# Diamondfan/CTC_pytorch

Hardware: AMD Instinct MI355X
Metric: acoustic frames/sec/GPU (train) + utterances/sec beam-decode (`decode` object), TIMIT 4x320 BiLSTM (higher is better)
Workload: dtype f32 via bf16x3 split-operand MFMA (f32 accumulate); 1 GPU; cfg2: 4x320 BiLSTM + BN + Linear(62) + CTC, B=32/GPU, T=800, F=40, dropout 0.1, Adam; global_batch=32, seq_len=800, parallelism=dp1, full_length_utterances=True, sync_bn=False

## Files before the change

ctc_pytorch_amd/_lib.py:

```python
import ctypes
import glob
import os
import subprocess

import torch

_HERE = os.path.dirname(os.path.abspath(__file__))
_CSRC = os.path.join(_HERE, "csrc")
SO_PATH = os.environ.get("CTCN_LIBCTCN") or os.path.join(_HERE, "libctcn.so")
_lib = None

c_void_p, c_int, c_float, c_double, c_size_t, c_u64 = (ctypes.c_void_p, ctypes.c_int, ctypes.c_float,
                                                      ctypes.c_double, ctypes.c_size_t, ctypes.c_uint64)

P, I, F, D, Z, U = c_void_p, c_int, c_float, c_double, c_size_t, c_u64
_SIGS = {
    "ctcn_version": (I, []),
    "ctcn_last_error": (ctypes.c_char_p, []),
    "ctcn_device_cus": (I, []),
    "ctcn_device_xcds": (I, []),
    "ctcn_set_option": (I, [ctypes.c_char_p, I]),
    "ctcn_get_option": (I, [ctypes.c_char_p]),
    "ctcn_option_name": (ctypes.c_char_p, [I]),
    "ctcn_set_status_buffer": (I, [P]),
    "ctcn_gemm": (I, [I, I, I, I, I, P, I, P, I, P, I, F, I, P, Z, P]),
    "ctcn_transpose01": (I, [P, P, I, I, I, P]),
    "ctcn_copy_strided4": (I, [P, P, I, I, I, I, Z, Z, Z, Z, P]),
    "ctcn_relu_fwd": (I, [P, P, Z, P]),
    "ctcn_relu_bwd": (I, [P, P, P, Z, P]),
    "ctcn_maxpool2d_fwd": (I, [P, P, P, Z, I, I, I, I, P]),
    "ctcn_maxpool2d_bwd": (I, [P, P, P, Z, I, I, I, I, P]),
    "ctcn_rnn_scratch_bytes": (Z, [I, I, I, I]),
    "ctcn_rnn_fwd": (I, [I, I, I, I, I, I, P, P, P, P, P, P, P, P, I, P, Z, P]),
    "ctcn_rnn_fwd_dropout": (I, [I, I, I, I, I, I, P, P, P, P, P, P, P, P, P, F, U, U, I, P, Z, P]),
    "ctcn_rnn_bwd": (I, [I, I, I, I, I, I, P, P, P, P, P, P, P, P, P, P, P, P, P, P, F, I, P, P, Z, P]),
    "ctcn_rnn_bwd_dropout": (I, [I, I, I, I, I, I, P, P, P, P, P, P, P, P, P, P, P, P, P, P, F, I, P, P, Z, P, F, U, U, P]),
    "ctcn_rnn_bwd_weights": (I, [I, I, I, I, I, I, P, P, P, P, P, P, P, P, F, I, ctypes.c_uint, P, Z, P]),
    "ctcn_bn_ws_bytes": (Z, [I, I, I]),
    "ctcn_bn_fwd_train": (I, [P, P, P, P, P, P, P, P, I, I, I, F, F, I, P, Z, P, P]),
    "ctcn_bn_fwd_eval": (I, [P, P, P, P, P, P, I, I, I, F, I, P]),
    "ctcn_bn_fwd_sums": (I, [P, P, I, I, I, P, Z, P]),
    "ctcn_bn_fwd_finish": (I, [P, P, P, P, P, P, P, P, P, D, I, I, I, F, F, I, P, P]),
    "ctcn_bn_bwd_sums": (I, [P, P, P, P, P, P, I, I, I, I, P, Z, P]),
    "ctcn_bn_bwd_finish": (I, [P, P, P, P, P, P, P, P, P, P, P, D, I, I, I, I, F, P, Z, P]),
    "ctcn_bn_bwd": (I, [P, P, P, P, P, P, P, P, P, I, I, I, I, F, P, Z, P]),
    "ctcn_bn_fwd_train_dropout": (I, [P, P, P, P, P, P, P, P, I, I, I, F, F, I, P, Z, P, P, F, U, U]),
    "ctcn_bn_bwd_dropout": (I, [P, P, P, P, P, P, P, P, P, I, I, I, I, F, P, Z, P, F, U, U]),
    "ctcn_dropout": (I, [P, P, Z, F, U, U, P]),
    "ctcn_conv2d_ws_bytes": (Z, [I] * 11),
    "ctcn_conv2d_fwd": (I, [P, P, P, P] + [I] * 11 + [P]),
    "ctcn_conv2d_bwd": (I, [P, P, P, P, P, P] + [I] * 11 + [F, P, Z, P]),
# ... 31 lines not shown
    "ctcn_diag_squat": (I, [I, I, I, ctypes.c_uint, P]),
    "ctcn_diag_pipeline_chunks": (I, [I, I, I, I, I, I, I, I, ctypes.c_uint]),
    "ctcn_rnn_last_kernel": (ctypes.c_char_p, [I]),
    "ctcn_levenshtein": (ctypes.c_longlong, [P, ctypes.c_longlong, P, ctypes.c_longlong]),
    "ctcn_join_tokens": (ctypes.c_longlong, [P, ctypes.c_longlong, P, I, P, P, P, I, I, P, ctypes.c_longlong, P]),
    "ctcn_beam_ws_bytes": (Z, [I, I, I, I]),
    "ctcn_beam_decode": (I, [P, I, P, P, D, I, I, P, P, P, P, I, I, I, P, Z, P]),
    "ctcn_beam_decode_nbest": (I, [P, I, P, P, D, I, I, I, P, P, P, P, P, I, I, I, P, Z, P]),
}


class RnnCall(ctypes.Structure):
    _fields_ = [("drop_p", ctypes.c_float), ("drop_seed", ctypes.c_uint64), ("drop_offset", ctypes.c_uint64), ("y_drop", ctypes.c_void_p),
                ("dy_tmp", ctypes.c_void_p), ("side_stream", ctypes.c_void_p), ("side_event", ctypes.c_void_p), ("side_ws", ctypes.c_void_p),
                ("side_ws_bytes", ctypes.c_size_t), ("xcd_allow", ctypes.c_uint), ("prelaunch_event", ctypes.c_void_p), ("status", ctypes.c_void_p),
                ("launched", ctypes.POINTER(ctypes.c_char_p))]


def sources():
    return sorted(glob.glob(os.path.join(_CSRC, "*.hip")))


def build(force=False, verbose=False):
    from concurrent.futures import ThreadPoolExecutor
    srcs = sources()
    hdrs = glob.glob(os.path.join(_CSRC, "*.h")) + [os.path.join(os.path.dirname(_HERE), "include", "ctcn.h")]
    hipcc = os.environ.get("HIPCC", "/opt/rocm/bin/hipcc")
    objdir = os.path.join(_CSRC, "_obj")
    os.makedirs(objdir, exist_ok=True)
    hdr_time = max(os.path.getmtime(h) for h in hdrs)
    flags = ["--offload-arch=gfx950", "-O3", "-std=c++17", "-fPIC"]
# ... 96 lines not shown
```

ctc_pytorch_amd/csrc/common.h:

```cpp
#pragma once
#include <hip/hip_runtime.h>
#include <stdarg.h>
#include <stdint.h>
#include <stdio.h>
#include <string.h>

#include "../../include/ctcn.h"

void ctcn_set_error(const char *fmt, ...);
int *ctcn_status_word(void);
int ctcn_opt_rnn_persistent(void);
int ctcn_transpose01_pair(const float *in0, const float *in1, float *out0, float *out1, int A, int B, int C, void *stream);
struct GemmPlanes {
  const float *A = nullptr; int lda = 0, M = 0, Ka = 0, transA = 0; void *ws_a = nullptr, *st_a = nullptr; bool a_valid = false;
  const float *B = nullptr; int ldb = 0, N = 0, Kb = 0, transB = 0, shift = 0; void *ws_b = nullptr, *st_b = nullptr; const void *bh = nullptr; bool b_valid = false;
  bool same_a = false, same_b = false;
};
int ctcn_gemm_on_xcds(int transA, int transB, int M, int N, int K, const float *A, int lda, const float *B, int ldb, float *C,
                      int ldc, float beta, int precision, void *ws, size_t ws_bytes, void *stream, unsigned xcd_allow, GemmPlanes *planes = nullptr);
int ctcn_gemm_shift_b(int M, int N, int K, const float *A, int lda, const float *B, int ldb, float *C, int ldc, float beta, int precision,
                      void *ws, size_t ws_bytes, void *stream, unsigned xcd_allow, int shift, GemmPlanes *planes = nullptr);
int ctcn_opt_handoff(void);
int ctcn_opt_poll_depth(void);
int ctcn_opt_bwd_scatter(void);
int ctcn_opt_handoff_tags(void);
int ctcn_opt_side_split_wgs(void);
int ctcn_opt_gemm_big_tiles(void);
int ctcn_opt_recurrence_only(void);

#define CTCN_REQUIRE(cond, ...)          \
  do {                                   \
    if (!(cond)) {                       \
// ... 65 lines not shown
```

ctc_pytorch_amd/csrc/core.hip:

```cpp
#include "common.h"

static thread_local char g_err[512] = "";

void ctcn_set_error(const char *fmt, ...) {
  va_list ap;
  va_start(ap, fmt);
  vsnprintf(g_err, sizeof(g_err), fmt, ap);
  va_end(ap);
}

extern "C" int ctcn_version(void) { return 100; }
extern "C" const char *ctcn_last_error(void) { return g_err; }
extern "C" int ctcn_device_cus(void) {
  int dev = 0, n = 0;
  if (hipGetDevice(&dev) != hipSuccess) return -1;
  if (hipDeviceGetAttribute(&n, hipDeviceAttributeMultiprocessorCount, dev) != hipSuccess) return -1;
  return n;
}

static int g_opt_rnn_persistent = 1;
static int g_opt_handoff = 1;
static int g_opt_poll_depth = 2;
static int g_opt_recurrence_only = 0;
static int g_opt_bwd_scatter = 1;
// ... 19 lines not shown
static int g_opt_conv_dbg = 0;
static int g_opt_rnn_rsv_nt = 0;
static int g_opt_gemm_bf16_single = 0;
static int g_opt_xcd_interleave = 1;
static int g_opt_bn_rows4 = 1;
static int g_opt_tn_splits_force = 0;
static int g_opt_tn_splits_xcd = 1;
static int g_opt_beam_generic_threads = 0;
static int g_opt_beam_bitonic = 1;
static int g_opt_beam_cand_global = 0;
static int g_opt_beam_occ2 = 0;
static int g_opt_beam_fast = 1;
static int g_opt_rnn_slow_items = 0;
static int g_opt_rnn_slow_exchange = 0;
static int g_opt_xcd_interleave_force = 0;
static int *g_status_dev = nullptr;

struct OptionRow { const char *name; int *var; int (*norm)(int); };
static const OptionRow k_options[] = {
  {"rnn_persistent", &g_opt_rnn_persistent, [](int value) -> int { return value; }},
  {"handoff", &g_opt_handoff, [](int value) -> int { return value; }},
  {"poll_depth", &g_opt_poll_depth, [](int value) -> int { return value; }},
  {"rnn_recurrence_only", &g_opt_recurrence_only, [](int value) -> int { return value ? 1 : 0; }},
  {"bwd_scatter", &g_opt_bwd_scatter, [](int value) -> int { return value ? 1 : 0; }},
  {"handoff_tags", &g_opt_handoff_tags, [](int value) -> int { return value ? 1 : 0; }},
  {"side_split_wgs", &g_opt_side_split_wgs, [](int value) -> int { return value < 1 ? 1 : (value > 16 ? 16 : value); }},
  {"gemm_big_tiles", &g_opt_gemm_big_tiles, [](int value) -> int { return value ? 1 : 0; }},
  {"beam_fast", &g_opt_beam_fast, [](int value) -> int { return value ? 1 : 0; }},
  {"conv_dbg", &g_opt_conv_dbg, [](int value) -> int { return value & 7; }},
  {"rnn_rsv_nt", &g_opt_rnn_rsv_nt, [](int value) -> int { return value ? 1 : 0; }},
// ... 12 lines not shown
  {"bwd_item_gather", &g_opt_bwd_item_gather, [](int value) -> int { return value < 0 ? 0 : (value > 2 ? 2 : value); }},
  {"bwd_poll_delay", &g_opt_bwd_poll_delay, [](int value) -> int { return value < 0 ? -1 : (value > 256 ? 256 : value); }},
  {"conv_mfma", &g_opt_conv_mfma, [](int value) -> int { return value ? 1 : 0; }},
  {"edit_wave", &g_opt_edit_wave, [](int value) -> int { return value ? 1 : 0; }},
  {"gemm_tn", &g_opt_gemm_tn, [](int value) -> int { return value != 0; }},
  {"rnn_fused_dropout", &g_opt_rnn_fused_dropout, [](int value) -> int { return value != 0; }},
  {"tag_poll_delay", &g_opt_tag_poll_delay, [](int value) -> int { return value < 0 ? 0 : (value > 64 ? 64 : value); }},
  {"rnn_fwd_tagged", &g_opt_rnn_fwd_tagged, [](int value) -> int { return value ? 1 : 0; }},
  {"rnn_mixed_slices", &g_opt_rnn_mixed_slices, [](int value) -> int { return value ? 1 : 0; }},
  {"gemm_pingpong", &g_opt_gemm_pingpong, [](int value) -> int { return value ? 1 : 0; }},
  {"gemm_a_inline", &g_opt_gemm_a_inline, [](int value) -> int { return value ? 1 : 0; }},
  {"gemm_dbg", &g_opt_gemm_dbg, [](int value) -> int { return value; }},
  {"gemm_tile256", &g_opt_gemm_tile256, [](int value) -> int { return value ? 1 : 0; }},
  {"xcd_interleave_force", &g_opt_xcd_interleave_force, [](int value) -> int { return value ? 1 : 0; }},
  {"rnn_slow_exchange", &g_opt_rnn_slow_exchange, [](int value) -> int { return value < 0 ? 0 : (value > 4096 ? 4096 : value); }},
  {"rnn_slow_items", &g_opt_rnn_slow_items, [](int value) -> int { return value < 0 ? 0 : (value > 4096 ? 4096 : value); }},
};
static const int k_noptions = (int)(sizeof(k_options) / sizeof(k_options[0]));
static const OptionRow *find_option(const char *name) {
  if (name)
    for (int i = 0; i < k_noptions; ++i)
      if (!strcmp(name, k_options[i].name)) return &k_options[i];
  return nullptr;
}
extern "C" int ctcn_set_option(const char *name, int value) {
  if (const OptionRow *o = find_option(name)) { *o->var = o->norm(value); return CTCN_OK; }
  ctcn_set_error("ctcn_set_option: unknown option %s", name ? name : "(null)");
  return CTCN_EINVAL;
}
extern "C" int ctcn_get_option(const char *name) {
// ... 15 lines not shown
```

ctc_pytorch_amd/csrc/gemm.hip:

```cpp
#include <algorithm>
#include <type_traits>

#include "common.h"

namespace {

constexpr int BM = 128, BN = 128, BK = 16, PAD = 4;

__device__ __forceinline__ void g2r_kc(const float *__restrict__ src, int ld, int r0, int R, int k0, int Kend,
                                       bool vec, int tid, float (&reg)[8]) {
#pragma unroll
  for (int j = 0; j < 2; ++j) {
    const int idx = tid + 256 * j;
    const int r = idx >> 2, kq = (idx & 3) * 4;
    const int gr = r0 + r, gk = k0 + kq;
    const float *p = src + (size_t)gr * ld + gk;
    if (vec && gr < R && gk + 3 < Kend) {
      const float4 v = *reinterpret_cast<const float4 *>(p);
      reg[4 * j + 0] = v.x; reg[4 * j + 1] = v.y; reg[4 * j + 2] = v.z; reg[4 * j + 3] = v.w;
    } else {
#pragma unroll
      for (int c = 0; c < 4; ++c) reg[4 * j + c] = (gr < R && gk + c < Kend) ? p[c] : 0.0f;
    }
  }
// ... 1623 lines not shown

}

static bool tn_eligible(int transA, int transB, int M, int N, int K, const float *A, int lda, const float *B, int ldb, int precision, const void *ws,
                        size_t ws_bytes) {
  return precision == 1 && transA && !transB && ws && ws_bytes >= 1024 && ctcn_get_option("gemm_tn") != 0 && M >= 128 && N >= 32 && K >= 1024 &&
         M % 4 == 0 && N % 4 == 0 && lda % 4 == 0 && ldb % 4 == 0 && ((uintptr_t)A & 15) == 0 && ((uintptr_t)B & 15) == 0 &&
         lda < (1 << 24) && ldb < (1 << 24);
}
static int gemm_core(int transA, int transB, int M, int N, int K, const float *A, int lda, const float *B, int ldb, float *C,
                     int ldc, float beta, int precision, void *ws, size_t ws_bytes, void *stream, unsigned xcd_allow, GemmPlanes *planes, int b_shift) {
  GemmPlanes scratch_planes;
  GemmPlanes &pl = planes ? *planes : scratch_planes;
  const bool want_same_a = pl.same_a, want_same_b = pl.same_b;
  pl.same_a = pl.same_b = false;
  CTCN_REQUIRE(precision == 0 || precision == 1, "ctcn_gemm: precision %d (0 = f32 MFMA, 1 = bf16x3 split MFMA)", precision);
  CTCN_REQUIRE(M > 0 && N > 0 && K >= 0, "ctcn_gemm: bad dims M=%d N=%d K=%d", M, N, K);
  CTCN_REQUIRE(A && B && C, "ctcn_gemm: null pointer");
  CTCN_REQUIRE(lda >= (transA ? M : K) && ldb >= (transB ? K : N) && ldc >= N, "ctcn_gemm: leading dim too small");
  hipStream_t st = (hipStream_t)stream;
  const int tiles_m = ceil_div(M, BM), tiles_n = ceil_div(N, BN);
  const int nt = tiles_m * tiles_n;
  int splits = 1;
  if (nt < 256 && K >= 512 && ws && ws_bytes >= (size_t)2 * M * N * sizeof(float)) {
    splits = ceil_div(512, nt);
    splits = min(splits, K / 256);
    splits = min(splits, (int)(ws_bytes / ((size_t)M * N * sizeof(float))));
    if (splits < 2) splits = 1;
  }
  int kchunk = K;
// ... 27 lines not shown
      int nq = 0;
      auto split = [&](const float *src, int ld, bool contraction_major, int rows, unsigned short *hi, unsigned short *lo, int shift) {
        if (!contraction_major) {
          const size_t total = (size_t)rows * (Kp / 4);
          hipLaunchKernelGGL(split_rows_kernel, dim3((unsigned)std::min((size_t)8192, ceil_div_z(total, 256))), dim3(256), 0, st, src, ld, rows, K, Kp, hi, lo);
        } else {
          if (xcd_allow)
            hipLaunchKernelGGL(split_transpose_queue_kernel, dim3(ctcn_opt_side_split_wgs() * ctcn_device_cus()), dim3(256), 0, st, src, ld, K, rows, Kp, hi, lo, ceil_div(rows, 64),
                               ceil_div(Kp, 64), xcd_allow, queue + (++nq), shift);
          else
            hipLaunchKernelGGL(split_transpose_kernel, dim3(ceil_div(rows, 64), ceil_div(Kp, 64)), dim3(256), 0, st, src, ld, K, rows, Kp, hi, lo, shift);
        }
      };
      const bool same_a = want_same_a && pl.a_valid && pl.A == A && pl.lda == lda && pl.M == M && pl.Ka == K && pl.transA == transA && pl.ws_a == ws &&
                          pl.st_a == (void *)st;
      const bool same_b = want_same_b && pl.b_valid && pl.B == B && pl.ldb == ldb && pl.N == N && pl.Kb == K && pl.transB == transB && pl.shift == b_shift &&
                          pl.ws_b == ws && pl.st_b == (void *)st && pl.bh == (const void *)bh;
      pl.B = B; pl.ldb = ldb; pl.N = N; pl.Kb = K; pl.transB = transB; pl.shift = b_shift; pl.ws_b = ws;
      pl.st_b = (void *)st; pl.bh = (const void *)bh; pl.b_valid = true;
      const int wnt256 = (N % 256 == 0 || (N > 512 && ceil_div(N, 256) * 256 - N <= N / 8)) ? 2 : 1;
      const bool use256 = !xcd_allow && ctcn_get_option("gemm_tile256") != 0 && M >= 1024 && N >= 96 &&
                          (long)ceil_div(M, 256) * ceil_div(N, 128 * wnt256) * 4 >= (long)ctcn_device_cus() * 3;
      const bool a_inline = use256 && !same_a && !transA && ctcn_get_option("gemm_a_inline") != 0 && K >= 32 && K % 4 == 0 && lda % 4 == 0 &&
                            ((uintptr_t)A & 15) == 0 && ceil_div(N, 128 * wnt256) <= 5;
      if (a_inline) {
        pl.a_valid = false;
        if (!same_b) split(B, ldb, transB == 0, N, bh, bl, b_shift);
        CTCN_LAUNCH_CHECK();
        const int lrc = wnt256 == 2 ? launch_planes256_af32<2>(st, M, N, K, Kp, A, lda, bh, bl, C, ldc, beta)
                                    : launch_planes256_af32<1>(st, M, N, K, Kp, A, lda, bh, bl, C, ldc, beta);
        if (lrc) return lrc;
        CTCN_LAUNCH_CHECK();
        return CTCN_OK;
      }
// ... 83 lines not shown
  } else {
    if (transA) { if (transB) LAUNCH(gemm_bf16x3_kernel, true, true); else LAUNCH(gemm_bf16x3_kernel, true, false); }
    else        { if (transB) LAUNCH(gemm_bf16x3_kernel, false, true); else LAUNCH(gemm_bf16x3_kernel, false, false); }
  }
#undef LAUNCH
  CTCN_LAUNCH_CHECK();
  if (splits > 1) {
    const size_t total = (size_t)M * N;
    const int blocks = (int)min((size_t)2048, ceil_div_z(total, 256));
    hipLaunchKernelGGL(splitk_reduce_kernel, dim3(blocks), dim3(256), 0, st, (const float *)ws, C, M, N, ldc, splits, beta);
    CTCN_LAUNCH_CHECK();
  }
  return CTCN_OK;
}

int ctcn_gemm_on_xcds(int transA, int transB, int M, int N, int K, const float *A, int lda, const float *B, int ldb, float *C,
                      int ldc, float beta, int precision, void *ws, size_t ws_bytes, void *stream, unsigned xcd_allow, GemmPlanes *planes) {
  return gemm_core(transA, transB, M, N, K, A, lda, B, ldb, C, ldc, beta, precision, ws, ws_bytes, stream, xcd_allow, planes, 0);
}

int ctcn_gemm_shift_b(int M, int N, int K, const float *A, int lda, const float *B, int ldb, float *C, int ldc, float beta, int precision,
                      void *ws, size_t ws_bytes, void *stream, unsigned xcd_allow, int shift, GemmPlanes *planes) {
  const int as = shift < 0 ? -shift : shift;
  CTCN_REQUIRE(as < K, "ctcn_gemm_shift_b: |shift| %d >= K %d", as, K);
  const int Kp = ceil_div(K, PBK) * PBK;
  const size_t plane_bytes = align_up(2 * ((size_t)M * Kp + (size_t)N * Kp) * sizeof(unsigned short), 256);
  const bool plane = precision == 1 && K >= 64 && ws && ws_bytes >= plane_bytes + 1024 &&
                     !tn_eligible(1, 0, M, N, K - as, A, lda, B, ldb, precision, ws, ws_bytes);
  if (!plane) {
    if (planes) planes->same_a = false;
// ... 67 lines not shown
```

ctc_pytorch_amd/csrc/rnn.hip:

```cpp
#include <algorithm>
#include <stdlib.h>

#include <atomic>

#include "common.h"
#include <type_traits>

namespace {

__device__ __forceinline__ float act_sigmoid(float x) { return __builtin_amdgcn_rcpf(1.0f + __builtin_amdgcn_exp2f(-1.4426950408889634f * x)); }
__device__ __forceinline__ float act_tanh(float x) {
  const float e = __builtin_amdgcn_exp2f(-2.8853900817779268f * fabsf(x));
  return copysignf((1.0f - e) * __builtin_amdgcn_rcpf(1.0f + e), x);
}

typedef __bf16 bf16x8_t __attribute__((ext_vector_type(8)));
union Bf16Pack { u32x4 u; bf16x8_t v; };
__device__ __forceinline__ void split8(const f32x4 &a, const f32x4 &b, bf16x8_t &hi, bf16x8_t &lo) {
  unsigned h[8], l[8];
#pragma unroll
  for (int e = 0; e < 8; ++e) {
    const float x = e < 4 ? a[e] : b[e - 4];
    h[e] = f2bf(x);
    l[e] = f2bf(x - __uint_as_float(h[e] << 16));
// ... 2377 lines not shown
                            float *aux, int precision, void *ws, size_t ws_bytes, void *stream) {
  return ctcn_rnn_fwd_ex(cell, T, B, I, H, dirs, x, w_ih0, w_hh0, w_ih1, w_hh1, y, gates, aux, precision, ws, ws_bytes, stream, nullptr);
}
extern "C" int ctcn_rnn_fwd_dropout(int cell, int T, int B, int I, int H, int dirs, const float *x, const float *w_ih0, const float *w_hh0,
                                    const float *w_ih1, const float *w_hh1, float *y, float *gates, float *aux, float *y_drop, float p, uint64_t seed,
                                    uint64_t offset, int precision, void *ws, size_t ws_bytes, void *stream) {
  CTCN_REQUIRE(y_drop && p >= 0.0f && p < 1.0f, "ctcn_rnn_fwd_dropout: y_drop NULL or p=%f outside [0,1)", (double)p);
  ctcn_rnn_call c = {};
  c.y_drop = y_drop; c.drop_p = p; c.drop_seed = seed; c.drop_offset = offset;
  return ctcn_rnn_fwd_ex(cell, T, B, I, H, dirs, x, w_ih0, w_hh0, w_ih1, w_hh1, y, gates, aux, precision, ws, ws_bytes, stream, &c);
}

static int rnn_bwd_gemms(int cell, int T, int B, int I, int H, int dirs, const float *x, const float *w_ih0, const float *w_ih1,
                         const float *y, const float *gates, const float *aux, float *dx, float *dw_ih0, float *dw_hh0, float *dw_ih1,
                         float *dw_hh1, float beta_w, int precision, bool weights, unsigned xcd_allow, void *ws, size_t ws_bytes,
                         void *stream) {
  const int G = gates_of(cell), GH = G * H, TB = T * B;
  const float *w_ih[2] = {w_ih0, w_ih1};
  float *dw_ih[2] = {dw_ih0, dw_ih1};
  float *dw_hh[2] = {dw_hh0, dw_hh1};
  GemmPlanes pl;
  bool dx_done = false;
  if (dx && dirs == 2) {
    StackedWih s;
    if (int rc = stack_w_ih(w_ih0, w_ih1, GH, I, ws, ws_bytes, (hipStream_t)stream, s)) return rc;
    if (s.w) {
      if (int rc = ctcn_gemm_on_xcds(0, 0, TB, I, 2 * GH, gates, 2 * GH, s.w, I, dx, I, 0.0f, precision, s.ws, s.ws_bytes, stream, xcd_allow)) return rc;
      dx_done = true;
    }
  }
  for (int d = 0; d < dirs; ++d) {
    const float *da = gates + (size_t)d * GH;
    const int ldg = dirs * GH;
    int rc;
    if (dx && !dx_done) {
      rc = ctcn_gemm_on_xcds(0, 0, TB, I, GH, da, ldg, w_ih[d], I, dx, I, d == 0 ? 0.0f : 1.0f, precision, ws, ws_bytes, stream, xcd_allow);
      if (rc) return rc;
    }
    if (!weights || !dw_ih[d]) continue;
    rc = ctcn_gemm_on_xcds(1, 0, GH, I, TB, da, ldg, x, I, dw_ih[d], I, beta_w, precision, ws, ws_bytes, stream, xcd_allow, &pl);
    if (rc) return rc;
    const int Kh = (T - 1) * B;
// ... 105 lines not shown
    if (done) note_kernel(1, "rnn_bwd_scatter", c.call);
  }
  return CTCN_OK;
}

static int bwd_per_timestep(BwdCall &c) {
  if (int rc = materialise_dropped_dy(c)) return rc;
  CTCN_HIP(hipMemsetAsync(c.a.state, 0, (size_t)c.B * c.dirs * c.H * sizeof(float), c.st()));
  const int kq4 = pick_kq4(c.GH, 16, 1, 5);
  note_kernel(1, "rnn_bwd_step", c.call);
  for (int s = 0; s < c.T; ++s) {
    c.a.step = s;
    launch_bwd(kq4, c.grid, c.st(), c.a);
  }
  return CTCN_OK;
}

extern "C" int ctcn_rnn_bwd_ex(int cell, int T, int B, int I, int H, int dirs, const float *x, const float *w_ih0,
                               const float *w_hh0, const float *w_ih1, const float *w_hh1, const float *y,
                               float *gates, float *aux, const float *dy, float *dx, float *dw_ih0, float *dw_hh0,
                               float *dw_ih1, float *dw_hh1, float beta_w, int precision, void *scratch, void *ws,
                               size_t ws_bytes, void *stream, const ctcn_rnn_call *call_p) {
  const ctcn_rnn_call &call = call_p ? *call_p : k_plain_call;
  CTCN_REQUIRE(!call.dy_tmp || (call.drop_p >= 0.0f && call.drop_p < 1.0f), "ctcn_rnn_bwd_ex: dropout p=%f outside [0,1)", (double)call.drop_p);
  CTCN_REQUIRE(cell >= 0 && cell <= 2, "ctcn_rnn_bwd: unknown cell %d", cell);
  CTCN_REQUIRE(T > 0 && B > 0 && I > 0 && H > 0 && (dirs == 1 || dirs == 2), "ctcn_rnn_bwd: bad dims");
  if (H % 4 != 0) { ctcn_set_error("ctcn_rnn_bwd: hidden size %d must be a multiple of 4", H); return CTCN_EUNSUPPORTED; }
  CTCN_REQUIRE(x && w_ih0 && w_hh0 && y && gates && dy && scratch, "ctcn_rnn_bwd: null pointer");
  CTCN_REQUIRE((dw_ih0 != nullptr) == (dw_hh0 != nullptr), "ctcn_rnn_bwd: dw_ih0 / dw_hh0 must both be given or both be NULL (weights deferred to ctcn_rnn_bwd_weights)");
  CTCN_REQUIRE(dirs == 1 || (w_ih1 && w_hh1 && (!dw_ih0 || (dw_ih1 && dw_hh1))), "ctcn_rnn_bwd: null pointer (reverse direction)");
// ... 1 lines not shown
  CTCN_REQUIRE((uintptr_t)gates % 16 == 0 && (uintptr_t)scratch % 16 == 0 && (cell == CTCN_CELL_TANH || (uintptr_t)aux % 16 == 0),
               "ctcn_rnn_bwd: gates / aux / scratch must be 16-byte aligned");
  BwdCall c = {cell, T, B, I, H, dirs, precision, dy, ws, ws_bytes, stream, call};
  c.G = gates_of(cell); c.GH = c.G * H;
  const int GH = c.GH;
  c.grid = dim3(ceil_div(H, 16), dirs, ceil_div(B, 16));
  c.status = call.status ? call.status : ctcn_status_word();
  c.fits32 = (size_t)T * B * dirs * GH * sizeof(float) < ((size_t)1 << 32);
  c.dy_dropped = call.dy_tmp == nullptr;
  c.prelaunch_event = call.prelaunch_event;
  c.nxd = ctcn_opt_handoff() ? ctcn_device_xcds() : 1;
  c.persistent = ctcn_opt_rnn_persistent() != 0; c.bwd_scatter = ctcn_opt_bwd_scatter() != 0; c.fused_dropout = ctcn_get_option("rnn_fused_dropout") != 0;
  c.handoff_tags = ctcn_opt_handoff_tags(); c.item_gather = ctcn_get_option("bwd_item_gather"); c.rsv_nt = ctcn_get_option("rnn_rsv_nt");
  c.poll_delay = ctcn_get_option("bwd_poll_delay"); c.slow_items = ctcn_get_option("rnn_slow_items"); c.slow_exchange = ctcn_get_option("rnn_slow_exchange");

  float *whhT = (float *)scratch;
  if (dirs == 2) {
    if (int rc = ctcn_transpose01_pair(w_hh0, w_hh1, whhT, whhT + (size_t)GH * H, GH, H, 1, stream)) return rc;
  } else if (int rc = ctcn_transpose01(w_hh0, whhT, GH, H, 1, stream)) {
    return rc;
  }
  RnnArgs &a = c.a;
  a.cell = cell; a.T = T; a.B = B; a.H = H; a.D = dirs; a.G = c.G; a.step = 0;
  a.w0 = whhT; a.w1 = whhT + (size_t)GH * H; a.y = const_cast<float *>(y); a.gates = gates; a.aux = aux; a.dy = dy;
  a.state = (float *)((char *)scratch + align_up((size_t)dirs * GH * H * sizeof(float), 256));

  bool done = false;
  if (c.persistent && T > 1) {
    const BwdPlan p = bwd_choose_formulation(c);
    Handoff h;
    if (p.feasible && carve_handoff(ws, ws_bytes, p.hx_bytes, p.fl_bytes, h))
      for (int mode = c.nxd > 1 ? 1 : 0; mode >= 0 && !done; --mode)
        if (int rc = bwd_try_persistent(c, p, h, mode, done)) return rc;
    if (!done)
      log_fallback("ctcn_rnn_bwd", T, B, H, dirs, !c.fits32 ? "a reserve tensor of 4 GB or more"
                                                       : (ceil_div(GH, 256) > 8 ? "gate width G*H above 2048" : "not co-resident / workspace too small"));
  }
  record_prelaunch(c);
  if (!done)
    if (int rc = bwd_per_timestep(c)) return rc;
  CTCN_LAUNCH_CHECK();

  if (ctcn_opt_recurrence_only()) return CTCN_OK;
  return rnn_bwd_gemms(cell, T, B, I, H, dirs, x, w_ih0, w_ih1, y, gates, aux, dx, dw_ih0, dw_hh0, dw_ih1, dw_hh1, beta_w, precision,
                       dw_ih0 != nullptr, 0u, ws, ws_bytes, stream);
}

extern "C" int ctcn_rnn_bwd_weights(int cell, int T, int B, int I, int H, int dirs, const float *x, const float *y, const float *gates,
                                    const float *aux, float *dw_ih0, float *dw_hh0, float *dw_ih1, float *dw_hh1, float beta_w,
                                    int precision, unsigned xcd_allow, void *ws, size_t ws_bytes, void *stream) {
  CTCN_REQUIRE(cell >= 0 && cell <= 2, "ctcn_rnn_bwd_weights: unknown cell %d", cell);
  CTCN_REQUIRE(T > 0 && B > 0 && I > 0 && H > 0 && (dirs == 1 || dirs == 2), "ctcn_rnn_bwd_weights: bad dims");
  CTCN_REQUIRE(x && y && gates && (dw_ih0 != nullptr) == (dw_hh0 != nullptr) && (dirs == 1 || (dw_ih1 != nullptr) == (dw_hh1 != nullptr)) &&
                   (dw_ih0 || (dirs == 2 && dw_ih1)), "ctcn_rnn_bwd_weights: null pointer");
  CTCN_REQUIRE(cell != CTCN_CELL_GRU || aux, "ctcn_rnn_bwd_weights: aux (d of the GRU n-gate) required");
  if (ctcn_opt_recurrence_only()) return CTCN_OK;
  return rnn_bwd_gemms(cell, T, B, I, H, dirs, x, nullptr, nullptr, y, gates, aux, nullptr, dw_ih0, dw_hh0, dw_ih1, dw_hh1, beta_w,
                       precision, true, xcd_allow, ws, ws_bytes, stream);
}

// ... 20 lines not shown
```

ctc_pytorch_amd/ops.py:

```python
import collections
import ctypes
import os
import numpy as np

import torch

from . import _lib

CELL = {"lstm": 0, "gru": 1, "tanh": 2}
GATES = {0: 4, 1: 3, 2: 1}

def _precision_from_env():
    v = os.environ.get("CTCN_PRECISION", "1").strip()
    if v not in ("0", "1"):
        raise ValueError("CTCN_PRECISION must be 0 (exact f32 MFMA) or 1 (bf16x3 split-operand MFMA), got %r" % v)
    return int(v)


DEFAULT_PRECISION = _precision_from_env()
_precision = [DEFAULT_PRECISION]


def set_precision(p):
    if int(p) not in (0, 1):
# ... 359 lines not shown
        piped = _side["enabled"] and _side["fwd_overlap"] and allow != 0 and dirs == 2 and T * B * H >= _side["min_items"]
        call = _lib.RnnCall()
        call.status = _lib.status_word(dev).data_ptr()
        if piped:
            st = _side_stream(dev)
            ev = _prelaunch_event(dev)
            w2, wp2, wn2 = _ws(x, tag="side")
            call.side_stream, call.side_event, call.side_ws, call.side_ws_bytes, call.xcd_allow = st.cuda_stream, ev.cuda_event, w2.data_ptr(), wn2, allow
        ctx.drop = None
        y_drop = None
        if training and drop_p > 0.0:
            y_drop = torch.empty_like(y)
            seed, off = _next_dropout_stream(y.numel())
            ctx.drop = (float(drop_p), seed, off)
            call.y_drop, call.drop_p, call.drop_seed, call.drop_offset = y_drop.data_ptr(), float(drop_p), seed, off
        launched = ctypes.c_char_p(None)
        call.launched = ctypes.pointer(launched)
        _lib.check(L.ctcn_rnn_fwd_ex(cell, T, B, I, H, dirs, _ptr(x), _ptr(ws[0]), _ptr(ws[1]), _ptr(ws[2]), _ptr(ws[3]),
                                     _ptr(y), _ptr(gates), _ptr(aux), get_precision(), wp, wn, _lib.stream_ptr(), ctypes.byref(call)), "rnn_fwd_ex")
        _count_kernel(launched.value)
        if T > 1 and B > 16 and (launched.value or b"") == b"rnn_fwd_step" and get_option("rnn_persistent"):
            _fallback_shapes.add((cell, H, dirs, B))
        if _debug_note[0] is not None:
            _debug_note[0]("rnn_fwd", dict(I=int(I), x=x.data_ptr(), gates=gates.data_ptr(), aux=aux.data_ptr() if aux is not None else 0, y=y.data_ptr(),
                                           y_drop=y_drop.data_ptr() if y_drop is not None else 0, ws=w.data_ptr(), w_ih=ws[0].data_ptr(), w_hh=ws[1].data_ptr()),
                           dict(x=x, y=y, gates=gates, aux=aux, y_drop=y_drop, w_ih=(ws[0], ws[2])))
        if piped:
            torch.cuda.current_stream(dev).wait_stream(st)
            for t in (x, gates, ws[0], ws[2]):
                if t is not None:
                    t.record_stream(st)
        ctx.cell, ctx.dims, ctx.has_aux = cell, (T, B, I, H, dirs), aux is not None
        ctx.early_ok = not _chunking[0]
        ctx.consumed = False
        ctx.counted = any(ctx.needs_input_grad)
        if ctx.counted:
            key = (dev.type, dev.index)
            _side["live"][key] = _side["live"].get(key, 0) + 1
        saved = [x, y, gates] + ([aux] if aux is not None else []) + [t for t in ws if t is not None]
        ctx.save_for_backward(*saved)
        return y if y_drop is None else y_drop

    @staticmethod
# ... 48 lines not shown
        small_split = (not side and not split_dirs and not chunk and into_flat and _side["enabled"] and _side["small_split"] and dirs == 2 and T > 1
                       and key not in _side["deferred"] and T * B * H < SMALL_SPLIT_MAX_ITEMS)
        if small_split:
            split_dirs = True
        above, ev = _side["deferred"].pop(key, None), None
        call = _lib.RnnCall()
        call.status = _lib.status_word(dev).data_ptr()
        if above is not None:
            ev = _prelaunch_event(dev)
            call.prelaunch_event = ev.cuda_event
        gd = None
        if ctx.drop is not None:
            p_, seed_, off_ = ctx.drop
            gd = torch.empty_like(gy)
            call.dy_tmp, call.drop_p, call.drop_seed, call.drop_offset = gd.data_ptr(), p_, seed_, off_
        launched = ctypes.c_char_p(None)
        call.launched = ctypes.pointer(launched)
        try:
            _lib.check(L.ctcn_rnn_bwd_ex(cell, T, B, I, H, dirs, _ptr(x), _ptr(w_ih0), _ptr(w_hh0), _ptr(w_ih1), _ptr(w_hh1),
                                         _ptr(y), _ptr(gates), _ptr(aux), _ptr(gy), _ptr(dx),
                                         null if (side or split_dirs) else _ptr(d_ih0), null if (side or split_dirs) else _ptr(d_hh0),
                                         null if (side or split_dirs) else _ptr(d_ih1), null if (side or split_dirs) else _ptr(d_hh1),
                                         1.0 if into_flat else 0.0, get_precision(), _ptr(scratch), wp, wn, _lib.stream_ptr(), ctypes.byref(call)), "rnn_bwd_ex")
        except Exception:
            if above is not None:
                _side["deferred"][key] = above
            raise
        _count_kernel(launched.value)
        if T > 1 and B > 16 and (launched.value or b"") == b"rnn_bwd_step" and get_option("rnn_persistent"):
            _fallback_shapes.add((cell, H, dirs, B))
# ... 836 lines not shown
```

include/ctcn.h:

```cpp
#ifndef CTCN_H
#define CTCN_H
#include <stddef.h>
#include <stdint.h>
#ifdef __cplusplus
extern "C" {
#endif

#define CTCN_OK 0
#define CTCN_EINVAL (-1)
#define CTCN_EHIP (-2)
#define CTCN_EUNSUPPORTED (-3)
#define CTCN_EWORKSPACE (-4)

#define CTCN_REDUCTION_NONE 0
#define CTCN_REDUCTION_MEAN 1
#define CTCN_REDUCTION_SUM 2

#define CTCN_CELL_LSTM 0
#define CTCN_CELL_GRU 1
#define CTCN_CELL_TANH 2

int ctcn_version(void);
const char *ctcn_last_error(void);
int ctcn_device_cus(void);
// ... 29 lines not shown
int ctcn_rnn_bwd_dropout(int cell, int T, int B, int I, int H, int dirs, const float *x, const float *w_ih0, const float *w_hh0,
                         const float *w_ih1, const float *w_hh1, const float *y, float *gates, float *aux, const float *dy, float *dx,
                         float *dw_ih0, float *dw_hh0, float *dw_ih1, float *dw_hh1, float beta_w, int precision, void *scratch, void *ws,
                         size_t ws_bytes, void *stream, float p, uint64_t seed, uint64_t offset, float *dy_tmp);
typedef struct ctcn_rnn_call {
  float drop_p;
  uint64_t drop_seed, drop_offset;
  float *y_drop;
  float *dy_tmp;
  void *side_stream, *side_event, *side_ws;
  size_t side_ws_bytes;
  unsigned xcd_allow;
  void *prelaunch_event;
  int *status;
  const char **launched;
} ctcn_rnn_call;
int ctcn_rnn_fwd_ex(int cell, int T, int B, int I, int H, int dirs, const float *x, const float *w_ih0, const float *w_hh0,
                    const float *w_ih1, const float *w_hh1, float *y, float *gates, float *aux, int precision, void *ws, size_t ws_bytes,
                    void *stream, const ctcn_rnn_call *call);
int ctcn_rnn_bwd_ex(int cell, int T, int B, int I, int H, int dirs, const float *x, const float *w_ih0, const float *w_hh0,
                    const float *w_ih1, const float *w_hh1, const float *y, float *gates, float *aux, const float *dy, float *dx,
                    float *dw_ih0, float *dw_hh0, float *dw_ih1, float *dw_hh1, float beta_w, int precision, void *scratch, void *ws,
                    size_t ws_bytes, void *stream, const ctcn_rnn_call *call);
int ctcn_rnn_bwd_weights(int cell, int T, int B, int I, int H, int dirs, const float *x, const float *y,
                         const float *gates, const float *aux, float *dw_ih0, float *dw_hh0, float *dw_ih1,
                         float *dw_hh1, float beta_w, int precision, unsigned xcd_allow, void *ws, size_t ws_bytes,
                         void *stream);

size_t ctcn_bn_ws_bytes(int outer, int C, int inner);
int ctcn_bn_fwd_train(const float *x, float *y, const float *gamma, const float *beta, float *running_mean,
                      float *running_var, float *save_mean, float *save_rstd, int outer, int C, int inner,
// ... 119 lines not shown
```

Measured before the change: 1.969 million frames/s.

## Precompute backward RNN weight transforms on side stream during forward

Adds a bwd-prep entry point that runs on a side stream during the forward pass. It transposes W_hh and splits the stacked W_ih into bf16 hi/lo planes. The backward pass then uses these prepared buffers through new ctcn_rnn_call fields, and the dx GEMM takes the external B planes, so the transpose and split work leaves the backward critical path. The prepared buffers are reused only when the weight tensor versions are unchanged. The cost is extra allocations per layer, a side-stream sync after the forward call, and more memory held between forward and backward.

New measurement: 1.969 million frames/s (median of 2 runs). About the same (-0.0%).

```diff
diff --git a/ctc_pytorch_amd/_lib.py b/ctc_pytorch_amd/_lib.py
--- a/ctc_pytorch_amd/_lib.py
+++ b/ctc_pytorch_amd/_lib.py
@@ -35,6 +35,8 @@
     "ctcn_rnn_fwd_dropout": (I, [I, I, I, I, I, I, P, P, P, P, P, P, P, P, P, F, U, U, I, P, Z, P]),
     "ctcn_rnn_bwd": (I, [I, I, I, I, I, I, P, P, P, P, P, P, P, P, P, P, P, P, P, P, F, I, P, P, Z, P]),
     "ctcn_rnn_bwd_dropout": (I, [I, I, I, I, I, I, P, P, P, P, P, P, P, P, P, P, P, P, P, P, F, I, P, P, Z, P, F, U, U, P]),
+    "ctcn_rnn_bwd_prep_bytes": (Z, [I, I, I, I, I]),
+    "ctcn_rnn_bwd_prep": (I, [I, I, I, I, P, P, P, P, P, P, P]),
     "ctcn_rnn_bwd_weights": (I, [I, I, I, I, I, I, P, P, P, P, P, P, P, P, F, I, ctypes.c_uint, P, Z, P]),
     "ctcn_bn_ws_bytes": (Z, [I, I, I]),
     "ctcn_bn_fwd_train": (I, [P, P, P, P, P, P, P, P, I, I, I, F, F, I, P, Z, P, P]),
@@ -96,7 +98,7 @@
     _fields_ = [("drop_p", ctypes.c_float), ("drop_seed", ctypes.c_uint64), ("drop_offset", ctypes.c_uint64), ("y_drop", ctypes.c_void_p),
                 ("dy_tmp", ctypes.c_void_p), ("side_stream", ctypes.c_void_p), ("side_event", ctypes.c_void_p), ("side_ws", ctypes.c_void_p),
                 ("side_ws_bytes", ctypes.c_size_t), ("xcd_allow", ctypes.c_uint), ("prelaunch_event", ctypes.c_void_p), ("status", ctypes.c_void_p),
-                ("launched", ctypes.POINTER(ctypes.c_char_p))]
+                ("launched", ctypes.POINTER(ctypes.c_char_p)), ("whh_t", ctypes.c_void_p), ("wih_planes", ctypes.c_void_p)]
 
 
 def sources():
diff --git a/ctc_pytorch_amd/csrc/common.h b/ctc_pytorch_amd/csrc/common.h
--- a/ctc_pytorch_amd/csrc/common.h
+++ b/ctc_pytorch_amd/csrc/common.h
@@ -15,7 +15,10 @@
   const float *A = nullptr; int lda = 0, M = 0, Ka = 0, transA = 0; void *ws_a = nullptr, *st_a = nullptr; bool a_valid = false;
   const float *B = nullptr; int ldb = 0, N = 0, Kb = 0, transB = 0, shift = 0; void *ws_b = nullptr, *st_b = nullptr; const void *bh = nullptr; bool b_valid = false;
   bool same_a = false, same_b = false;
+  const unsigned short *ext_bh = nullptr, *ext_bl = nullptr;
 };
+size_t ctcn_gemm_b_plane_elems(int N, int K);
+int ctcn_gemm_split_b(const float *B, int ldb, int N, int K, unsigned short *hi, unsigned short *lo, void *stream);
 int ctcn_gemm_on_xcds(int transA, int transB, int M, int N, int K, const float *A, int lda, const float *B, int ldb, float *C,
                       int ldc, float beta, int precision, void *ws, size_t ws_bytes, void *stream, unsigned xcd_allow, GemmPlanes *planes = nullptr);
 int ctcn_gemm_shift_b(int M, int N, int K, const float *A, int lda, const float *B, int ldb, float *C, int ldc, float beta, int precision,
diff --git a/ctc_pytorch_amd/csrc/core.hip b/ctc_pytorch_amd/csrc/core.hip
--- a/ctc_pytorch_amd/csrc/core.hip
+++ b/ctc_pytorch_amd/csrc/core.hip
@@ -57,6 +57,7 @@
 static int g_opt_rnn_slow_items = 0;
 static int g_opt_rnn_slow_exchange = 0;
 static int g_opt_xcd_interleave_force = 0;
+static int g_opt_bwd_weight_prep = 1;
 static int *g_status_dev = nullptr;
 
 struct OptionRow { const char *name; int *var; int (*norm)(int); };
@@ -99,6 +100,7 @@
   {"gemm_tile256", &g_opt_gemm_tile256, [](int value) -> int { return value ? 1 : 0; }},
   {"xcd_interleave_force", &g_opt_xcd_interleave_force, [](int value) -> int { return value ? 1 : 0; }},
   {"rnn_slow_exchange", &g_opt_rnn_slow_exchange, [](int value) -> int { return value < 0 ? 0 : (value > 4096 ? 4096 : value); }},
+  {"bwd_weight_prep", &g_opt_bwd_weight_prep, [](int value) -> int { return value ? 1 : 0; }},
   {"rnn_slow_items", &g_opt_rnn_slow_items, [](int value) -> int { return value < 0 ? 0 : (value > 4096 ? 4096 : value); }},
 };
 static const int k_noptions = (int)(sizeof(k_options) / sizeof(k_options[0]));
diff --git a/ctc_pytorch_amd/csrc/gemm.hip b/ctc_pytorch_amd/csrc/gemm.hip
--- a/ctc_pytorch_amd/csrc/gemm.hip
+++ b/ctc_pytorch_amd/csrc/gemm.hip
@@ -1661,6 +1661,8 @@
   GemmPlanes &pl = planes ? *planes : scratch_planes;
   const bool want_same_a = pl.same_a, want_same_b = pl.same_b;
   pl.same_a = pl.same_b = false;
+  const unsigned short *ext_bh = pl.ext_bh, *ext_bl = pl.ext_bl;
+  pl.ext_bh = pl.ext_bl = nullptr;
   CTCN_REQUIRE(precision == 0 || precision == 1, "ctcn_gemm: precision %d (0 = f32 MFMA, 1 = bf16x3 split MFMA)", precision);
   CTCN_REQUIRE(M > 0 && N > 0 && K >= 0, "ctcn_gemm: bad dims M=%d N=%d K=%d", M, N, K);
   CTCN_REQUIRE(A && B && C, "ctcn_gemm: null pointer");
@@ -1718,10 +1720,12 @@
       };
       const bool same_a = want_same_a && pl.a_valid && pl.A == A && pl.lda == lda && pl.M == M && pl.Ka == K && pl.transA == transA && pl.ws_a == ws &&
                           pl.st_a == (void *)st;
-      const bool same_b = want_same_b && pl.b_valid && pl.B == B && pl.ldb == ldb && pl.N == N && pl.Kb == K && pl.transB == transB && pl.shift == b_shift &&
-                          pl.ws_b == ws && pl.st_b == (void *)st && pl.bh == (const void *)bh;
+      const bool ext_b = ext_bh && ext_bl && !transB && b_shift == 0 && !xcd_allow;
+      if (ext_b) { bh = const_cast<unsigned short *>(ext_bh); bl = const_cast<unsigned short *>(ext_bl); }
+      const bool same_b = ext_b || (want_same_b && pl.b_valid && pl.B == B && pl.ldb == ldb && pl.N == N && pl.Kb == K && pl.transB == transB && pl.shift == b_shift &&
+                                    pl.ws_b == ws && pl.st_b == (void *)st && pl.bh == (const void *)bh);
       pl.B = B; pl.ldb = ldb; pl.N = N; pl.Kb = K; pl.transB = transB; pl.shift = b_shift; pl.ws_b = ws;
-      pl.st_b = (void *)st; pl.bh = (const void *)bh; pl.b_valid = true;
+      pl.st_b = (void *)st; pl.bh = (const void *)bh; pl.b_valid = !ext_b;
       const int wnt256 = (N % 256 == 0 || (N > 512 && ceil_div(N, 256) * 256 - N <= N / 8)) ? 2 : 1;
       const bool use256 = !xcd_allow && ctcn_get_option("gemm_tile256") != 0 && M >= 1024 && N >= 96 &&
                           (long)ceil_div(M, 256) * ceil_div(N, 128 * wnt256) * 4 >= (long)ctcn_device_cus() * 3;
@@ -1835,6 +1839,15 @@
   return CTCN_OK;
 }
 
+size_t ctcn_gemm_b_plane_elems(int N, int K) { return (size_t)N * (ceil_div(K, PBK) * PBK); }
+int ctcn_gemm_split_b(const float *B, int ldb, int N, int K, unsigned short *hi, unsigned short *lo, void *stream) {
+  CTCN_REQUIRE(B && hi && lo && N > 0 && K > 0 && ldb >= N, "ctcn_gemm_split_b: bad args");
+  const int Kp = ceil_div(K, PBK) * PBK;
+  hipLaunchKernelGGL(split_transpose_kernel, dim3(ceil_div(N, 64), ceil_div(Kp, 64)), dim3(256), 0, (hipStream_t)stream, B, ldb, K, N, Kp, hi, lo, 0);
+  CTCN_LAUNCH_CHECK();
+  return CTCN_OK;
+}
+
 int ctcn_gemm_on_xcds(int transA, int transB, int M, int N, int K, const float *A, int lda, const float *B, int ldb, float *C,
                       int ldc, float beta, int precision, void *ws, size_t ws_bytes, void *stream, unsigned xcd_allow, GemmPlanes *planes) {
   return gemm_core(transA, transB, M, N, K, A, lda, B, ldb, C, ldc, beta, precision, ws, ws_bytes, stream, xcd_allow, planes, 0);
diff --git a/ctc_pytorch_amd/csrc/rnn.hip b/ctc_pytorch_amd/csrc/rnn.hip
--- a/ctc_pytorch_amd/csrc/rnn.hip
+++ b/ctc_pytorch_amd/csrc/rnn.hip
@@ -2415,7 +2415,7 @@
 static int rnn_bwd_gemms(int cell, int T, int B, int I, int H, int dirs, const float *x, const float *w_ih0, const float *w_ih1,
                          const float *y, const float *gates, const float *aux, float *dx, float *dw_ih0, float *dw_hh0, float *dw_ih1,
                          float *dw_hh1, float beta_w, int precision, bool weights, unsigned xcd_allow, void *ws, size_t ws_bytes,
-                         void *stream) {
+                         void *stream, const void *wih_planes = nullptr) {
   const int G = gates_of(cell), GH = G * H, TB = T * B;
   const float *w_ih[2] = {w_ih0, w_ih1};
   float *dw_ih[2] = {dw_ih0, dw_ih1};
@@ -2426,7 +2426,12 @@
     StackedWih s;
     if (int rc = stack_w_ih(w_ih0, w_ih1, GH, I, ws, ws_bytes, (hipStream_t)stream, s)) return rc;
     if (s.w) {
-      if (int rc = ctcn_gemm_on_xcds(0, 0, TB, I, 2 * GH, gates, 2 * GH, s.w, I, dx, I, 0.0f, precision, s.ws, s.ws_bytes, stream, xcd_allow)) return rc;
+      GemmPlanes pdx;
+      if (wih_planes && s.w == w_ih0 && precision == 1) {
+        pdx.ext_bh = (const unsigned short *)wih_planes;
+        pdx.ext_bl = pdx.ext_bh + ctcn_gemm_b_plane_elems(I, 2 * GH);
+      }
+      if (int rc = ctcn_gemm_on_xcds(0, 0, TB, I, 2 * GH, gates, 2 * GH, s.w, I, dx, I, 0.0f, precision, s.ws, s.ws_bytes, stream, xcd_allow, &pdx)) return rc;
       dx_done = true;
     }
   }
@@ -2562,6 +2567,11 @@
     launch_bwd(kq4, c.grid, c.st(), c.a);
   }
   return CTCN_OK;
+}
+
+static int transpose_w_hh(const float *w_hh0, const float *w_hh1, float *out, int GH, int H, int dirs, void *stream) {
+  if (dirs == 2) return ctcn_transpose01_pair(w_hh0, w_hh1, out, out + (size_t)GH * H, GH, H, 1, stream);
+  return ctcn_transpose01(w_hh0, out, GH, H, 1, stream);
 }
 
 extern "C" int ctcn_rnn_bwd_ex(int cell, int T, int B, int I, int H, int dirs, const float *x, const float *w_ih0,
@@ -2593,12 +2603,12 @@
   c.handoff_tags = ctcn_opt_handoff_tags(); c.item_gather = ctcn_get_option("bwd_item_gather"); c.rsv_nt = ctcn_get_option("rnn_rsv_nt");
   c.poll_delay = ctcn_get_option("bwd_poll_delay"); c.slow_items = ctcn_get_option("rnn_slow_items"); c.slow_exchange = ctcn_get_option("rnn_slow_exchange");
 
-  float *whhT = (float *)scratch;
-  if (dirs == 2) {
-    if (int rc = ctcn_transpose01_pair(w_hh0, w_hh1, whhT, whhT + (size_t)GH * H, GH, H, 1, stream)) return rc;
-  } else if (int rc = ctcn_transpose01(w_hh0, whhT, GH, H, 1, stream)) {
-    return rc;
-  }
+  const float *whhT = call.whh_t;
+  if (!whhT) {
+    if (int rc = transpose_w_hh(w_hh0, w_hh1, (float *)scratch, GH, H, dirs, stream)) return rc;
+    whhT = (const float *)scratch;
+  }
+  CTCN_REQUIRE((uintptr_t)whhT % 16 == 0, "ctcn_rnn_bwd: ctcn_rnn_call.whh_t must be 16-byte aligned");
   RnnArgs &a = c.a;
   a.cell = cell; a.T = T; a.B = B; a.H = H; a.D = dirs; a.G = c.G; a.step = 0;
   a.w0 = whhT; a.w1 = whhT + (size_t)GH * H; a.y = const_cast<float *>(y); a.gates = gates; a.aux = aux; a.dy = dy;
@@ -2622,7 +2632,25 @@
 
   if (ctcn_opt_recurrence_only()) return CTCN_OK;
   return rnn_bwd_gemms(cell, T, B, I, H, dirs, x, w_ih0, w_ih1, y, gates, aux, dx, dw_ih0, dw_hh0, dw_ih1, dw_hh1, beta_w, precision,
-                       dw_ih0 != nullptr, 0u, ws, ws_bytes, stream);
+                       dw_ih0 != nullptr, 0u, ws, ws_bytes, stream, call.wih_planes);
+}
+
+extern "C" size_t ctcn_rnn_bwd_prep_bytes(int cell, int I, int H, int dirs, int which) {
+  if (cell < 0 || cell > 2 || I <= 0 || H <= 0 || (dirs != 1 && dirs != 2) || (which != 0 && which != 1)) return 0;
+  const int GH = gates_of(cell) * H;
+  if (which == 0) return align_up((size_t)dirs * GH * H * sizeof(float), 256);
+  return dirs == 2 ? align_up(2 * ctcn_gemm_b_plane_elems(I, 2 * GH) * sizeof(unsigned short), 256) : 0;
+}
+extern "C" int ctcn_rnn_bwd_prep(int cell, int I, int H, int dirs, const float *w_ih0, const float *w_hh0, const float *w_ih1, const float *w_hh1,
+                                 float *whh_t, void *wih_planes, void *stream) {
+  CTCN_REQUIRE(cell >= 0 && cell <= 2 && I > 0 && H > 0 && (dirs == 1 || dirs == 2), "ctcn_rnn_bwd_prep: bad dims");
+  CTCN_REQUIRE(w_hh0 && whh_t && (dirs == 1 || w_hh1), "ctcn_rnn_bwd_prep: null pointer");
+  const int GH = gates_of(cell) * H;
+  if (int rc = transpose_w_hh(w_hh0, w_hh1, whh_t, GH, H, dirs, stream)) return rc;
+  if (!wih_planes) return CTCN_OK;
+  CTCN_REQUIRE(dirs == 2 && w_ih0 && w_ih1 == w_ih0 + (size_t)GH * I, "ctcn_rnn_bwd_prep: wih_planes needs two directions with w_ih1 directly behind w_ih0");
+  unsigned short *hi = (unsigned short *)wih_planes;
+  return ctcn_gemm_split_b(w_ih0, I, I, 2 * GH, hi, hi + ctcn_gemm_b_plane_elems(I, 2 * GH), stream);
 }
 
 extern "C" int ctcn_rnn_bwd_weights(int cell, int T, int B, int I, int H, int dirs, const float *x, const float *y, const float *gates,
diff --git a/ctc_pytorch_amd/ops.py b/ctc_pytorch_amd/ops.py
--- a/ctc_pytorch_amd/ops.py
+++ b/ctc_pytorch_amd/ops.py
@@ -397,6 +397,9 @@
             seed, off = _next_dropout_stream(y.numel())
             ctx.drop = (float(drop_p), seed, off)
             call.y_drop, call.drop_p, call.drop_seed, call.drop_offset = y_drop.data_ptr(), float(drop_p), seed, off
+        prep = (training and any(ctx.needs_input_grad) and _side["enabled"] and not _chunking[0] and T > 1 and get_option("bwd_weight_prep") != 0)
+        if prep:
+            _side_stream(dev).wait_stream(torch.cuda.current_stream(dev))
         launched = ctypes.c_char_p(None)
         call.launched = ctypes.pointer(launched)
         _lib.check(L.ctcn_rnn_fwd_ex(cell, T, B, I, H, dirs, _ptr(x), _ptr(ws[0]), _ptr(ws[1]), _ptr(ws[2]), _ptr(ws[3]),
@@ -408,8 +411,21 @@
             _debug_note[0]("rnn_fwd", dict(I=int(I), x=x.data_ptr(), gates=gates.data_ptr(), aux=aux.data_ptr() if aux is not None else 0, y=y.data_ptr(),
                                            y_drop=y_drop.data_ptr() if y_drop is not None else 0, ws=w.data_ptr(), w_ih=ws[0].data_ptr(), w_hh=ws[1].data_ptr()),
                            dict(x=x, y=y, gates=gates, aux=aux, y_drop=y_drop, w_ih=(ws[0], ws[2])))
+        ctx.prep = None
+        if prep:
+            st = _side_stream(dev)
+            stacked = dirs == 2 and get_precision() == 1 and ws[2].data_ptr() == ws[0].data_ptr() + 4 * G * H * I
+            whh_t = torch.empty(L.ctcn_rnn_bwd_prep_bytes(cell, I, H, dirs, 0), dtype=torch.uint8, device=dev)
+            planes = torch.empty(L.ctcn_rnn_bwd_prep_bytes(cell, I, H, dirs, 1), dtype=torch.uint8, device=dev) if stacked else None
+            _lib.check(L.ctcn_rnn_bwd_prep(cell, I, H, dirs, _ptr(ws[0]), _ptr(ws[1]), _ptr(ws[2]), _ptr(ws[3]), _ptr(whh_t), _ptr(planes),
+                                           st.cuda_stream), "rnn_bwd_prep")
+            for t in (whh_t, planes) + tuple(ws):
+                if t is not None:
+                    t.record_stream(st)
+            ctx.prep = (whh_t, planes, [t._version for t in ws if t is not None])
+        if piped or prep:
+            torch.cuda.current_stream(dev).wait_stream(st)
         if piped:
-            torch.cuda.current_stream(dev).wait_stream(st)
             for t in (x, gates, ws[0], ws[2]):
                 if t is not None:
                     t.record_stream(st)
@@ -488,6 +504,9 @@
             p_, seed_, off_ = ctx.drop
             gd = torch.empty_like(gy)
             call.dy_tmp, call.drop_p, call.drop_seed, call.drop_offset = gd.data_ptr(), p_, seed_, off_
+        if ctx.prep is not None and ctx.prep[2] == [t._version for t in wts]:
+            call.whh_t = ctx.prep[0].data_ptr()
+            call.wih_planes = ctx.prep[1].data_ptr() if ctx.prep[1] is not None else None
         launched = ctypes.c_char_p(None)
         call.launched = ctypes.pointer(launched)
         try:
diff --git a/include/ctcn.h b/include/ctcn.h
--- a/include/ctcn.h
+++ b/include/ctcn.h
@@ -67,7 +67,12 @@
   void *prelaunch_event;
   int *status;
   const char **launched;
+  const float *whh_t;
+  const void *wih_planes;
 } ctcn_rnn_call;
+size_t ctcn_rnn_bwd_prep_bytes(int cell, int I, int H, int dirs, int which);
+int ctcn_rnn_bwd_prep(int cell, int I, int H, int dirs, const float *w_ih0, const float *w_hh0, const float *w_ih1, const float *w_hh1,
+                      float *whh_t, void *wih_planes, void *stream);
 int ctcn_rnn_fwd_ex(int cell, int T, int B, int I, int H, int dirs, const float *x, const float *w_ih0, const float *w_hh0,
                     const float *w_ih1, const float *w_hh1, float *y, float *gates, float *aux, int precision, void *ws, size_t ws_bytes,
                     void *stream, const ctcn_rnn_call *call);
```
